# deeppowers/deeppowers

Hardware: AMD Instinct MI355X
Metric: ciphertext-mul/s (N=4096, 4 RNS limbs) (higher is better)
Workload: dtype u64

## Files before the change

### deeppowers_amd/csrc/ctx_tables.h

```cpp
#pragma once
#include <cstring>
#include <vector>

#include "devtables.h"
#include "ntt_core.h"
#include "ntt_quarters.h"
#include "tables.h"

namespace dpfhe {

static_assert(sizeof(TwShoup) == 16 && sizeof(TwFold) == 16 && sizeof(TwF64) == 16, "the twiddle slots of every class share one stride");
struct alignas(16) TwBytes { u64 lo, hi; };
constexpr size_t kTwSize = sizeof(TwBytes);

template <class Tw> inline TwBytes tw_bytes(const Tw& t) { static_assert(sizeof(Tw) == sizeof(TwBytes), "slot size"); TwBytes r; std::memcpy(&r, &t, sizeof r); return r; }
inline TwBytes class_tw(LimbClass k, u64 w, u64 q) {
    if (k == kClassFold) return tw_bytes(h_tw_fold(w, q));
    if (k == kClassFoldScaled) return tw_bytes(h_tw_fold_scaled(w, q, fold_scaled_shift(q)));
    if (k == kClassF64 || k == kClassF64Wide) return tw_bytes(h_make_tw<TwF64>(w, q));
    return tw_bytes(h_make_tw<TwShoup>(w, q));
}
inline InvLast<TwBytes> class_last(LimbClass k, u64 w_last, u64 w_ninv, u64 q) { return InvLast<TwBytes>{class_tw(k, w_last, q), class_tw(k, w_ninv, q)}; }
inline void pack_table(unsigned char* dst, const std::vector<u64>& words, LimbClass k, u64 q, int logn_tab, int loge) {
    std::vector<TwBytes> t(words.size());
// ... 34 lines not shown
        const u64 sinv = cls == kClassFoldScaled ? h_powmod((1ull << fold_scaled_shift(q)) % q, q - 2, q) : 1;
        reinterpret_cast<InvLast<TwBytes>*>(&blob[m.o_last2])[l] = class_last(cls, h_mulmod(t.w_last, sinv, q), h_mulmod(t.lc.ninv, sinv, q), q);
    }
    return blob;
}
template <class Arith>
inline DevTables<Arith> mixed_view(const unsigned char* b, const MixedLayout& m, size_t L) {
    typedef typename Arith::Tw Tw;
    DevTables<Arith> tb{};
    tb.lc = reinterpret_cast<const LimbConst*>(b + m.o_lc);
    tb.fwd = reinterpret_cast<const Tw*>(b + m.o_fwd); tb.inv = reinterpret_cast<const Tw*>(b + m.o_inv);
    tb.fwd4 = reinterpret_cast<const Tw*>(b + m.o_fwd4); tb.inv4 = reinterpret_cast<const Tw*>(b + m.o_inv4);
    tb.last = reinterpret_cast<const InvLast<Tw>*>(b + m.o_last);
    tb.last2 = reinterpret_cast<const InvLast<Tw>*>(b + m.o_last2);
    tb.n_sub = 1;
    tb.n_limbs = (int)L;
    return tb;
}
inline bool ctx_limb_classes(int log2n, const std::vector<HostLimbTables>& ht, bool fold, unsigned char limb_cls[16]) {
    if (fold || ht.size() > 16 || log2n < 8 || log2n > 14) return false;
    bool any_fast = false;
    for (size_t l = 0; l < ht.size(); ++l) { limb_cls[l] = (unsigned char)limb_class(ht[l].lc.q); any_fast = any_fast || limb_cls[l] != kClassShoup; }
    return any_fast;
}

struct CtxLayout {
    int log_n1, log_n2, loge_ntt;
    size_t n_sub, n2;
    bool split, two_geo, halves, quarters;
    size_t o_lc, o_fwd4, o_inv4, o_fwd, o_inv, o_last, o_top_fwd, o_top_inv, o_top_last, o_resc, o_hfwd, o_hinv, o_htop_fwd, o_htop_last,
           o_qfwd, o_qinv, o_qtop_fwd, o_qtop_inv, o_qtop_last, total;
};
inline CtxLayout ctx_layout(int log2n, size_t L, bool fold) {
    auto up = [](size_t x) { return (x + 255) & ~(size_t)255; };
    CtxLayout m;
    m.log_n1 = split_log_n1(log2n); m.log_n2 = log2n - m.log_n1;
    m.n_sub = (size_t)1 << m.log_n1; m.n2 = (size_t)1 << m.log_n2;
    m.loge_ntt = ntt_loge(m.log_n2);
    m.split = m.log_n1 > 0; m.two_geo = !m.split && m.loge_ntt != kFusedLoge;
    m.halves = log2n == 13 && fold;
    m.quarters = log2n == 14 && fold;
    const size_t n_sub = m.n_sub, tab = L * ((size_t)1 << log2n) * kTwSize;
    m.o_lc = 0; m.o_fwd4 = up(m.o_lc + L * sizeof(LimbConst)); m.o_inv4 = up(m.o_fwd4 + tab);
    m.o_fwd = m.two_geo ? up(m.o_inv4 + tab) : m.o_fwd4; m.o_inv = m.two_geo ? up(m.o_fwd + tab) : m.o_inv4;
    m.o_last = up(m.o_inv + tab); m.o_top_fwd = up(m.o_last + L * n_sub * 2 * kTwSize); m.o_top_inv = up(m.o_top_fwd + L * n_sub * kTwSize);
    m.o_top_last = up(m.o_top_inv + L * n_sub * kTwSize); m.o_resc = up(m.o_top_last + L * 2 * kTwSize);
// ... 86 lines not shown
```

### deeppowers_amd/csrc/devtables.h

```cpp
#pragma once
#include "modarith.h"

namespace dpfhe {

struct QuartersTop;

constexpr int ntt_loge(int ) { return 4; }
constexpr int kMaxLog2N = 16;
constexpr int kSplitLog2N2 = 12;
constexpr int split_log_n1(int log2n) { return log2n > 14 ? log2n - kSplitLog2N2 : 0; }
constexpr int kFusedLoge = 4;

template <class Tw>
struct InvLast {
    Tw w_last;
    Tw w_ninv;
};

template <class Arith>
struct DevTables {
    const typename Arith::Tw* fwd;
    const typename Arith::Tw* inv;
    const typename Arith::Tw* fwd4;
    const typename Arith::Tw* inv4;
    const typename Arith::Tw* top_fwd;
    const typename Arith::Tw* top_inv;
    const InvLast<typename Arith::Tw>* top_last;
    int n_sub;
    const typename Arith::Tw* hfwd;
    const typename Arith::Tw* hinv;
    const typename Arith::Tw* htop_fwd;
    const InvLast<typename Arith::Tw>* htop_last;
    const typename Arith::Tw* qfwd;
    const typename Arith::Tw* qinv;
    const struct QuartersTop* qtop_fwd;
    const typename Arith::Tw* qtop_inv;
    const InvLast<typename Arith::Tw>* qtop_last;
    const InvLast<typename Arith::Tw>* last;
    const InvLast<typename Arith::Tw>* last2;
    const LimbConst* lc;
    int n_limbs;
    int n_active;
    unsigned long long active_map;
};

template <class TB>
DPF_HD void block_item_limb(const TB& tb, size_t blk, size_t& item, int& limb) {
    if (tb.n_active) {
        item = blk / (unsigned)tb.n_active;
        limb = (int)((tb.active_map >> (4u * (unsigned)(blk % (unsigned)tb.n_active))) & 15u);
    } else {
        item = blk / (unsigned)tb.n_limbs;
        limb = (int)(blk % (unsigned)tb.n_limbs);
    }
}

struct MixedTables {
    const void* fwd;
    const void* inv;
    const void* last;
    const LimbConst* lc;
    int n_limbs;
// ... 12 lines not shown
```

### deeppowers_amd/csrc/dpfhe_cabi.hip

```cpp
#include <dlfcn.h>
#include <hip/hip_runtime.h>

#include <algorithm>
#include <atomic>
#include <cstdio>
#include <cstdlib>
#include <cstring>
#include <mutex>
#include <new>
#include <string>
#include <vector>

#include "../../include/dpfhe.h"
#include "base_ext.h"
#include "compact.h"
#include "ctx_tables.h"
#include "encode.h"
#include "expand.h"
#include "noise.h"
#include "plain_add.h"
#include "kernels_large.h"
#include "kernels_misc.h"
#include "launch.h"
#include "tables.h"
// ... 35 lines not shown
    return a0 < b0 + nb && b0 < a0 + na;
}
static inline bool overlaps(const uint64_t* a, size_t na, const uint64_t* b, size_t nb) { return overlaps_bytes(a, na * 8, b, nb * 8); }

static inline bool misaligned(const void* p) { return (reinterpret_cast<uintptr_t>(p) & 15) != 0; }
static const size_t kMaxGrid = 0x7fffffff;

struct dpfhe_ctx {
    uint32_t log2n = 0, n_limbs = 0;
    int device = 0;
    bool fold = false;
    int n_cu = 256;
    std::vector<uint64_t> moduli;
    uint64_t p_special = 0;
    void* d_blob = nullptr;
    const LimbConst* lc = nullptr;
    const RescaleConst* d_rescale = nullptr;
    DevTables<ShoupArith> shoup{};
    DevTables<FoldArith> foldt{};
    bool classes = false;
    int uniform_cls = kClassShoup;
    unsigned char limb_cls[16] = {};
    unsigned long long cls_map = 0;
    void* class_blob = nullptr;
    DevTables<FoldArith> cls_fold{};
    DevTables<F64Arith> cls_f64{};
    DevTables<FoldScaledArith> cls_fscaled{};
    DevTables<F64WideArith> cls_f64w{};
    DevTables<ShoupArith> cls_shoup{};
    MixedTables mixed{};
    struct ScratchArena { hipStream_t stream; u64* p; size_t words; uint64_t last_use; };
    std::vector<ScratchArena> scratch_arenas;
    uint64_t scratch_clock = 0;
    std::mutex scratch_mutex;
    std::atomic<int> ct_mul_variant{0};
    dpfhe_tune_info tune{};
    mutable std::mutex tune_mutex;
    std::atomic<size_t> scratch_limit_words{(size_t)1024 << 17};
};


static const char* const kCtMulVariantNames[kCtMulVariants] = {"quad", "dual"};
static const float kTuneMargin = 0.97f;

__global__ __launch_bounds__(256) void tune_fill_kernel(u64* __restrict__ p, size_t n) {
    for (size_t i = (size_t)blockIdx.x * 256 + threadIdx.x; i < n; i += (size_t)gridDim.x * 256)
// ... 161 lines not shown
    c->d_rescale = reinterpret_cast<const RescaleConst*>(d + lay.o_resc);
    if (fold) c->foldt = ctx_view<FoldArith>(d, lay, L);
    else c->shoup = ctx_view<ShoupArith>(d, lay, L);
    if (ctx_limb_classes((int)log2_n, ht, fold, c->limb_cls)) {
        const MixedLayout m = mixed_layout((int)log2_n, L);
        const std::vector<unsigned char> mb = build_class_blob((int)log2_n, ht, c->limb_cls);
        for (size_t l = 0; l < L; ++l) c->cls_map |= (unsigned long long)c->limb_cls[l] << (4 * l);
        if (int rc = upload(c->class_blob, mb, "dpfhe_ctx_create: class table upload")) return rc;
        const unsigned char* b = static_cast<const unsigned char*>(c->class_blob);
        c->cls_fold = mixed_view<FoldArith>(b, m, L);
        c->cls_f64 = mixed_view<F64Arith>(b, m, L);
        c->cls_fscaled = mixed_view<FoldScaledArith>(b, m, L);
        c->cls_f64w = mixed_view<F64WideArith>(b, m, L);
        c->cls_shoup = mixed_view<ShoupArith>(b, m, L);
        c->mixed.fwd = b + m.o_fwd; c->mixed.inv = b + m.o_inv; c->mixed.last = b + m.o_last;
        c->mixed.lc = reinterpret_cast<const LimbConst*>(b + m.o_lc);
        c->mixed.n_limbs = (int)L;
        c->mixed.cls_map = c->cls_map;
        c->classes = true;
        bool same = true;
        for (size_t l = 1; l < L; ++l) same = same && c->limb_cls[l] == c->limb_cls[0];
        if (same) c->uniform_cls = c->limb_cls[0];
    }
    tune_at_create(c);
    (void)hipSetDevice(prev);
    *out = c;
    return DPFHE_SUCCESS;
}

extern "C" int dpfhe_ctx_destroy(dpfhe_ctx* c) {
    if (!c) return DPFHE_SUCCESS;
    if (c->d_blob) (void)hipFree(c->d_blob);
    if (c->class_blob) (void)hipFree(c->class_blob);
    for (auto& a : c->scratch_arenas) if (a.p) (void)hipFree(a.p);
    delete c;
    return DPFHE_SUCCESS;
}
extern "C" int dpfhe_ctx_set_scratch_limit(dpfhe_ctx* c, size_t mib) {
    if (!c) return fail(DPFHE_INVALID_ARGUMENT, "dpfhe_ctx_set_scratch_limit", "null context");
    if (mib == 0 || mib > ((size_t)1 << 20)) return fail(DPFHE_INVALID_ARGUMENT, "dpfhe_ctx_set_scratch_limit", "limit must be in [1 MiB, 1 TiB]");
    c->scratch_limit_words.store(mib << 17, std::memory_order_relaxed);
    return DPFHE_SUCCESS;
}
extern "C" uint32_t dpfhe_ctx_log2n(const dpfhe_ctx* c) { return c ? c->log2n : 0; }
extern "C" uint32_t dpfhe_ctx_limbs(const dpfhe_ctx* c) { return c ? c->n_limbs : 0; }
extern "C" int dpfhe_ctx_uses_fold(const dpfhe_ctx* c) { return c && c->fold ? 1 : 0; }
extern "C" int dpfhe_ctx_limb_class(const dpfhe_ctx* c, uint32_t limb) {
    if (!c || limb >= c->n_limbs) return -1;
    if (c->classes) return (int)c->limb_cls[limb];
    return c->fold ? DPFHE_ARITH_FOLD : DPFHE_ARITH_SHOUP;
}
static_assert(DPFHE_ARITH_SHOUP == kClassShoup && DPFHE_ARITH_FOLD == kClassFold && DPFHE_ARITH_F64 == kClassF64 && DPFHE_ARITH_FOLD_SCALED == kClassFoldScaled &&
              DPFHE_ARITH_F64_WIDE == kClassF64Wide, "dpfhe.h <-> tables.h");

constexpr int kMatvecWpt2 = 2, kMatvecWpt4 = 1;
constexpr int kMatvecWd = 1;
// ... 1489 lines not shown
```

### deeppowers_amd/csrc/kernels.h

```cpp
#pragma once
#include <hip/hip_runtime.h>

#include "devtables.h"
#include "launch.h"
#include "ntt_core.h"
#include "ntt_top.h"

namespace dpfhe {

__device__ __forceinline__ void lds_barrier() { __syncthreads(); }
__device__ __forceinline__ void wave_sync() {
    __builtin_amdgcn_fence(__ATOMIC_ACQ_REL, "wavefront");
    __builtin_amdgcn_wave_barrier();
}
template <class G, int X, bool FWD>
__device__ __forceinline__ void exch_sync_before_write() {
    if constexpr (G::exch_wave_local(X)) {
        wave_sync();
    } else {
        constexpr bool first = FWD ? X == 0 : G::highest_cross_wave_exchange() == X;
        if constexpr (!first) lds_barrier();
    }
}
template <class G, int X>
// ... 509 lines not shown
        InvChain2<BI, B::NPH - 1, kInvIn>::run(tid, D0, D1, lds, lds + W, twi, last, lc);
        B::inv_canon(D0, lc);
        B::template store_top<true>(tid, D0, dst);
        B::inv_canon(D1, lc);
        B::template store_top<true>(tid, D1, dst + cstride);
        asm volatile("" : "+v"(tid));
        lds_barrier();
        InvChain<BI, B::NPH - 1, kInvIn>::run(tid, D2, lds, twi, last, lc);
        B::inv_canon(D2, lc);
        B::template store_top<true>(tid, D2, dst + 2 * cstride);
    }
}

constexpr int kTraceWords = 12;
template <bool TRACE>
__device__ __forceinline__ u64 trace_stamp(u64 dep) {
    u64 t = 0;
    if constexpr (TRACE) asm volatile("s_memrealtime %0\n\ts_waitcnt lgkmcnt(0)" : "=s"(t) : "v"(dep) : "memory");
    return t;
}
template <class Arith, int LOGN, int LOGE, bool TRACE = false, bool OUT_NTT = false>
__global__ __launch_bounds__(1 << (LOGN - LOGE), 2) void ct_mul_quad_kernel(u64* __restrict__ out3, const u64* __restrict__ a2,
                                                                         const u64* __restrict__ b2, DevTables<Arith> tb, u64* __restrict__ trace = nullptr) {
    typedef NttBody<Arith, LOGN, LOGE> B;
    static_assert(B::kLazyProducts && LOGE == kFusedLoge, "a policy with lazy products (ntt_core.h prod), fused twiddle layout");
    typedef NttBody<Arith, LOGN, LOGE, 0, kUnit, true> BI;
    constexpr bool kScaledProducts = Arith::kFoldCore && !Arith::kFold;
    constexpr int E = B::E, N = B::G::N, W = B::G::lds_words();
    __shared__ __attribute__((aligned(16))) u64 lds[2 * W];
    const int tid = threadIdx.x;
    const u64 ts0 = trace_stamp<TRACE>((u64)tid);
    const size_t L = (size_t)tb.n_limbs;
    size_t bi;
    int limb;
    block_item_limb(tb, blockIdx.x, bi, limb);
    const LimbConst lc = tb.lc[limb];
    const u64* src_a = a2 + ((bi * 2) * L + limb) * N;
    const u64* src_b = b2 + ((bi * 2) * L + limb) * N;
    u64* dst = out3 + ((bi * 3) * L + limb) * N;
    const size_t cstride = L * N;
    const InvLast<typename B::Tw> last = kScaledProducts ? tb.last2[limb] : tb.last[limb];
    constexpr int kInvIn = B::kProdInvIn;
    u64 x[E], y[E], z[E], w[E];
    const u64 ts_p = trace_stamp<TRACE>((u64)(uintptr_t)src_a ^ (u64)lc.q);
    B::template load_top<true>(tid, x, src_a);
    const u64 ts_x = trace_stamp<TRACE>((u64)tid);
    B::template load_top<true>(tid, y, src_b);
    B::template load_top<true>(tid, z, src_a + cstride);
    B::template load_top<true>(tid, w, src_b + cstride);
    const u64 ts_i = trace_stamp<TRACE>((u64)tid);
    const u64 ts1 = trace_stamp<TRACE>(x[0]);
    const u64 ts_xl = trace_stamp<TRACE>(x[E - 1]);
    FwdChain4<B, 0>::run(tid, x, y, z, w, lds, lds + W, tb.fwd4 + (size_t)limb * N, lc);
    B::prod_partner(y, lc);
    B::prod_partner(w, lc);
    const u64 ts2 = trace_stamp<TRACE>(w[E - 1]);
#pragma unroll
    for (int k = 0; k < E; ++k) {
        const u64 a0 = x[k], b0 = y[k], a1 = z[k], b1 = w[k];
        B::tensor(a0, a1, b0, b1, x[k], y[k], z[k], lc);
    }
    const u64 ts3 = trace_stamp<TRACE>(z[E - 1]);
    if constexpr (OUT_NTT) {
        static_assert(Arith::kFold && !TRACE, "the pinned primes (the products of a scaled-fold limb carry the scale twice)");
#pragma unroll
        for (int k = 0; k < E; ++k) { x[k] = FoldArith::canon_small(x[k], lc); y[k] = FoldArith::canon_small(y[k], lc); z[k] = FoldArith::canon_small(z[k], lc); }
        B::store_bot(tid, x, dst);
        B::store_bot(tid, y, dst + cstride);
        B::store_bot(tid, z, dst + 2 * cstride);
        return;
    }
    constexpr bool kNtStore = true;
    InvChain3<BI, B::NPH - 1, kInvIn>::run(tid, x, y, z, lds, lds + W, tb.inv4 + (size_t)limb * N, last, lc);
    const u64 ts4 = trace_stamp<TRACE>(z[E - 1]);
    B::inv_canon(x, lc);
    B::template store_top<kNtStore>(tid, x, dst);
    B::inv_canon(y, lc);
    B::template store_top<kNtStore>(tid, y, dst + cstride);
    B::inv_canon(z, lc);
    B::template store_top<kNtStore>(tid, z, dst + 2 * cstride);
    if constexpr (TRACE) {
        const u64 ts5 = trace_stamp<TRACE>((u64)tid);
        asm volatile("s_waitcnt vmcnt(0)" ::: "memory");
        const u64 ts6 = trace_stamp<TRACE>((u64)tid);
        if (tid == 0) {
            unsigned hw, xcc;
            asm volatile("s_getreg_b32 %0, hwreg(HW_REG_HW_ID)" : "=s"(hw));
            asm volatile("s_getreg_b32 %0, hwreg(HW_REG_XCC_ID)" : "=s"(xcc));
            u64* t = trace + (size_t)blockIdx.x * kTraceWords;
            t[0] = ts0; t[1] = ts1; t[2] = ts2; t[3] = ts3; t[4] = ts4; t[5] = ts5; t[6] = ts6;
            t[7] = (u64)hw | ((u64)xcc << 32);
            t[8] = ts_p; t[9] = ts_x; t[10] = ts_i; t[11] = ts_xl;
        }
    }
}

// ... 408 lines not shown
```

### deeppowers_amd/csrc/modarith.h

```cpp
#pragma once
#include <stdint.h>

#if defined(__HIPCC__)
#define DPF_HD __host__ __device__ __forceinline__
#else
#define DPF_HD inline __attribute__((always_inline))
#endif

namespace dpfhe {

typedef uint64_t u64;
typedef uint32_t u32;

#if defined(DPFHE_EMU_CHECK) && !defined(__HIPCC__)
extern long g_emu_overflows;
#define DPFHE_EMU_ASSERT(cond) do { if (!(cond)) ++g_emu_overflows; } while (0)
#else
#define DPFHE_EMU_ASSERT(cond) do { } while (0)
#endif

struct LimbConst {
    u64 q;
    u64 d;
    u64 ninv;
// ... 112 lines not shown
        DPFHE_EMU_ASSERT(((a | b | as | bs) >> 30) == 0);
        const u64 H = mad32(y1, bs, mad32(y0, b, 0));
        u32 two30 = 1u << 30;
#if defined(__HIP_DEVICE_COMPILE__)
        asm("s_mov_b32 %0, 0x40000000" : "=s"(two30));
#endif
        const u64 L = mad32(y1, as, mad32(y0, a, mad32((u32)H, two30, 0)));
        const u64 R = mad32((u32)(H >> 32), 4 * (u32)c.d, L);
        return reduce(R, c);
    }
    static DPF_HD u64 mul_tw_add(u64 y, const Tw& t, const LimbConst& c, u64 addend) {
        const u32 y0 = (u32)y, y1 = (u32)(y >> 32);
        const u32 a = (u32)t.w, b = (u32)(t.w >> 32), as = (u32)t.ws, bs = (u32)(t.ws >> 32);
        DPFHE_EMU_ASSERT(((a | b | as | bs) >> 30) == 0);
        DPFHE_EMU_ASSERT((unsigned __int128)addend + ((unsigned __int128)y0 << 30) + ((unsigned __int128)y1 << 30) + (1ull << 62) + (1ull << 54) < ((unsigned __int128)1 << 64));
        const u64 H = mad32(y1, bs, mad32(y0, b, 0));
        u32 two30 = 1u << 30;
#if defined(__HIP_DEVICE_COMPILE__)
        asm("s_mov_b32 %0, 0x40000000" : "=s"(two30));
#endif
        const u64 L = mad32(y1, as, mad32(y0, a, mad32((u32)H, two30, addend)));
        const u64 R = mad32((u32)(H >> 32), 4 * (u32)c.d, L);
        return reduce(R, c);
    }
    static DPF_HD Tw prod_tw(u64 b, const LimbConst& c) {
        DPFHE_EMU_ASSERT(b < (1ull << 60) + (1ull << 29));
        const u32 lo = (u32)b;
        u32 a = lo & 0x3fffffffu, bh = (u32)(b >> 30), t29 = (u32)(b >> 29), bl = lo & 0x1fffffffu;
#if defined(__HIP_DEVICE_COMPILE__)
        asm("" : "+v"(a), "+v"(bh), "+v"(t29), "+v"(bl));
#endif
        const u64 bs = add_hi32(mad32(t29, 2 * (u32)c.d, 0), bl);
        u32 as = (u32)bs & 0x3fffffffu, bsh = (u32)(bs >> 30);
#if defined(__HIP_DEVICE_COMPILE__)
        asm("" : "+v"(as), "+v"(bsh));
#endif
        Tw t;
        t.w = (u64)a | ((u64)bh << 32);
        t.ws = (u64)as | ((u64)bsh << 32);
        return t;
    }
    static DPF_HD bool ptw_fits(u32 y0, u32 y1, u32 a, u32 b, u32 as, u32 bs, u64 addend, u32 d) {
        typedef unsigned __int128 u128;
        const u128 H = (u128)y0 * b + (u128)y1 * bs;
        const u128 L = (u128)((u32)(u64)H) * (1u << 30) + (u128)y0 * a + (u128)y1 * as + addend;
        return (H >> 64) == 0 && ((L + (u128)(u32)((u64)H >> 32) * (4 * d)) >> 64) == 0;
// ... 153 lines not shown
```

### deeppowers_amd/csrc/ntt_core.h

```cpp
#pragma once
#include "modarith.h"

namespace dpfhe {

#if defined(DPFHE_EMU_CHECK) && !defined(__HIPCC__)
inline u64 chk_add(u64 a, u64 b) { if ((unsigned __int128)a + b >> 64) ++g_emu_overflows; return a + b; }
inline u64 chk_sub_add(u64 a, u64 b, u64 off) {
    __int128 v = (__int128)a - (__int128)b + (__int128)off;
    if (v < 0 || (v >> 64)) ++g_emu_overflows;
    return a - b + off;
}
inline u64 chk_shl1_add_sub(u64 a, u64 c, u64 s) {
    __int128 v = 2 * (__int128)a + (__int128)c - (__int128)s;
    if (v < 0 || (v >> 64) || ((unsigned __int128)2 * a + c) >> 64) ++g_emu_overflows;
    return shl1_add(a, c) - s;
}
#else
DPF_HD u64 chk_shl1_add_sub(u64 a, u64 c, u64 s) { return shl1_add(a, c) - s; }
DPF_HD u64 chk_add(u64 a, u64 b) { return a + b; }
DPF_HD u64 chk_sub_add(u64 a, u64 b, u64 off) { return a - b + off; }
#endif

struct Phase {
    int c;
    int b;
    int r;
};

constexpr int geo_nph(int logn, int loge) { return (logn + loge - 1) / loge; }
constexpr Phase geo_phase(int logn, int loge, int p) {
    int rem = logn, top = logn, r = 0;
    for (int i = 0; i <= p; ++i) {
        int left = geo_nph(logn, loge) - i;
        r = (rem + left - 1) / left;
        top = rem;
        rem -= r;
    }
    int b = top - r;
    int c = b < (logn - loge) ? b : (logn - loge);
    return Phase{c, b, r};
// ... 137 lines not shown
    int bnd[E] = {};
    for (int k = 0; k < E; ++k) bnd[k] = in_bound;
    for (int u = 0; u < r; ++u) {
        const int bit = 1 << (lb_top - u);
        for (int k = 0; k < E; ++k) {
            if (k & bit) continue;
            int A = bnd[k];
            const int Y = bnd[k | bit];
            if (A + Y / 4 + 1 > kFuseLimit || (u == r - 1 && A > kRedB && 2 * A + 2 * kUnit > out_cap)) { p.red_a[u][k] = true; A = kRedB; }
            bnd[k] = kRedB;
            bnd[k | bit] = 2 * A + 2 * kUnit;
        }
    }
    int mx = 0;
    for (int k = 0; k < E; ++k) {
        if (bnd[k] > out_cap) { p.red_end[k] = true; bnd[k] = kRedB; }
        p.out[k] = bnd[k];
        if (bnd[k] > mx) mx = bnd[k];
    }
    p.out_bound = mx;
    return p;
}

constexpr int kF64Red = kUnit / 2 + 1, kF64Tw = kUnit;
template <int LOGE>
struct F64CtPlan {
    bool red_y[LOGE][1 << LOGE];
    bool red_a[LOGE][1 << LOGE];
    bool red_end[1 << LOGE];
    int out_bound;
};
template <int LOGE>
constexpr F64CtPlan<LOGE> make_f64_ct_plan(int lb_top, int r, int in_bound, int out_cap, int cap) {
    F64CtPlan<LOGE> p{};
    constexpr int E = 1 << LOGE;
    int bnd[E] = {};
    for (int k = 0; k < E; ++k) bnd[k] = in_bound;
    for (int u = 0; u < r; ++u) {
        const int bit = 1 << (lb_top - u);
        for (int k = 0; k < E; ++k) {
            if (k & bit) continue;
            int A = bnd[k], Y = bnd[k | bit];
            if (Y > cap) { p.red_y[u][k] = true; Y = kF64Red; }
            if (A + kF64Tw > 4 * cap) { p.red_a[u][k] = true; A = kF64Red; }
            bnd[k] = bnd[k | bit] = A + kF64Tw;
        }
// ... 18 lines not shown
    int bnd[E] = {};
    for (int k = 0; k < E; ++k) bnd[k] = in_bound;
    for (int u = 0; u < r; ++u) {
        const int bit = 1 << (lb0 + u);
        for (int k = 0; k < E; ++k) {
            if (k & bit) continue;
            int bx = bnd[k], by = bnd[k | bit];
            if (bx + by > cap) {
                if (bx > kF64Red) { p.red[u][k] = true; bx = kF64Red; }
                if (by > kF64Red) { p.red[u][k | bit] = true; by = kF64Red; }
            }
            bnd[k] = (last_all_mul && u == r - 1) ? kF64Tw : bx + by;
            bnd[k | bit] = kF64Tw;
        }
    }
    for (int k = 0; k < E; ++k) {
        p.red_end[k] = bnd[k] > out_bound;
        if (p.red_end[k]) bnd[k] = kF64Red;
    }
    return p;
}

constexpr int kSubInvOut = 7 * kUnit;
template <class Arith, int LOGN, int LOGE, int SUB = 0, int FWD_IN = (SUB ? kCtfMid : kUnit), bool RAW_INV = false>
struct NttBody {
    typedef Geo<LOGN, LOGE> G;
    typedef typename Arith::Tw Tw;
    static constexpr int E = G::E, T = G::T, NPH = G::NPH;
    static_assert(FWD_IN >= kUnit && FWD_IN <= kCtfMid && (!SUB || FWD_IN == kCtfMid), "forward input bound: canonical ... the phase hand-over bound");

    static DPF_HD unsigned row_base(int k) {
        constexpr int kReach = 4096 / (T * 8) > 0 ? 4096 / (T * 8) : 1;
        unsigned b = (unsigned)(k / kReach * kReach) * T;
#if defined(__HIP_DEVICE_COMPILE__)
        asm("" : "+s"(b));
#endif
        return b;
    }
    template <bool NT, class V>
    static DPF_HD V ld_stream(const V* p) {
#if defined(__HIP_DEVICE_COMPILE__)
        if (NT) return __builtin_nontemporal_load(p);
#endif
        return *p;
    }
    template <bool NT, class V>
    static DPF_HD void st_stream(V* p, V v) {
#if defined(__HIP_DEVICE_COMPILE__)
        if (NT) { __builtin_nontemporal_store(v, p); return; }
#endif
        *p = v;
    }
// ... 230 lines not shown
        int in = kUnit;
        for (int i = 0; i < P; ++i) {
            const Phase pi = G::phase(i);
            in = make_f64_ct_plan<LOGE>(pi.b - pi.c + pi.r - 1, pi.r, in, 2 * kF64Cap, kF64Cap).out_bound;
        }
        return make_f64_ct_plan<LOGE>(ph.b - ph.c + ph.r - 1, ph.r, in, (P == NPH - 1) ? kF64Cap : 2 * kF64Cap, kF64Cap);
    }
    template <int P, int IN>
    static constexpr F64GsPlan<LOGE> f64_gs_plan() {
        constexpr Phase ph = G::phase(P);
        constexpr int mid = kF64Cap / 2 > 2 * kUnit ? 2 * kUnit : kF64Cap / 2;
        return make_f64_gs_plan<LOGE>(ph.b - ph.c, ph.r, (P == NPH - 1) ? IN : mid, (P == 0) ? kF64Cap : mid, P == 0, kF64Cap);
    }
    template <int P>
    static constexpr CtfPlan<LOGE> ctf_plan() {
        constexpr Phase ph = G::phase(P);
        int in = FWD_IN;
        for (int i = 0; i < P; ++i) {
            const Phase pi = G::phase(i);
            in = make_ctf_plan<LOGE>(pi.b - pi.c + pi.r - 1, pi.r, in, kCtfMid).out_bound;
        }
        return make_ctf_plan<LOGE>(ph.b - ph.c + ph.r - 1, ph.r, in, (P == NPH - 1) ? kWord : kCtfMid);
    }
    static constexpr int kFwdOutBound = Arith::kFoldCore ? ctf_plan<NPH - 1>().out_bound : Arith::kF64 ? f64_ct_plan<NPH - 1>().out_bound : 4 * kUnit;
    static_assert(!Arith::kFoldCore || kFwdOutBound <= kLimitPartner, "lazy forward outputs must satisfy mul60's bound");

    static constexpr bool kConverts = Arith::kF64 || (Arith::kFoldCore && !Arith::kFold);
    static_assert(!kConverts || !SUB, "the halves form is FoldArith's");

    static DPF_HD void enter(u64 (&x)[E], const LimbConst& lc) {
        if constexpr (kConverts) {
#pragma clang loop unroll(full)
            for (int k = 0; k < E; ++k) x[k] = Arith::enter(x[k], lc);
        }
    }
    template <int P>
    static DPF_HD void fwd_phase_r(u64 (&x)[E], const TwRegs& twr, const LimbConst& lc_in) {
        constexpr Phase ph = G::phase(P);
        const auto& lc = Arith::ntt_lc(lc_in);
        if constexpr (P == 0) enter(x, lc_in);
        const u64 two_q = 2 * lc.q;
        if constexpr (Arith::kF64) {
            constexpr F64CtPlan<LOGE> plan = f64_ct_plan<P>();
            const double q = Arith::qd(lc), qi = Arith::qinv(lc);
#pragma clang loop unroll(full)
            for (int u = 0; u < ph.r; ++u) {
                const int lb = ph.b + ph.r - 1 - u - ph.c;
#pragma clang loop unroll(full)
                for (int k = 0; k < E; ++k) {
                    if (k & (1 << lb)) continue;
                    const int kk = k | (1 << lb);
                    const Tw& w = twr[u][k >> (lb + 1)];
                    double a = Arith::f(x[k]), y = Arith::f(x[kk]);
                    if (plan.red_a[u][k]) a = Arith::reduce(a, q, qi);
                    if (plan.red_y[u][k]) y = Arith::reduce(y, q, qi);
                    const double t = Arith::mulmod(y, w.w, w.wq, q);
                    x[k] = Arith::b(a + t);
                    x[kk] = Arith::b(a - t);
                }
            }
#pragma clang loop unroll(full)
            for (int k = 0; k < E; ++k)
                if (plan.red_end[k]) x[k] = Arith::b(Arith::reduce(Arith::f(x[k]), q, qi));
        } else if constexpr (Arith::kFoldCore) {
            constexpr CtfPlan<LOGE> plan = ctf_plan<P>();
#pragma clang loop unroll(full)
            for (int u = 0; u < ph.r; ++u) {
                const int lb = ph.b + ph.r - 1 - u - ph.c;
#pragma clang loop unroll(full)
                for (int k = 0; k < E; ++k) {
                    if (k & (1 << lb)) continue;
                    const int kk = k | (1 << lb);
                    u64 a = x[k];
                    if (plan.red_a[u][k]) a = FoldArith::reduce(a, lc);
                    const u64 s = FoldArith::mul_tw_add(x[kk], twr[u][k >> (lb + 1)], lc, a);
                    x[k] = s;
                    x[kk] = chk_shl1_add_sub(a, two_q, s);
                }
            }
#pragma clang loop unroll(full)
            for (int k = 0; k < E; ++k)
                if (plan.red_end[k]) x[k] = FoldArith::reduce(x[k], lc);
        } else {
#pragma clang loop unroll(full)
            for (int u = 0; u < ph.r; ++u) {
                const int lb = ph.b + ph.r - 1 - u - ph.c;
#pragma clang loop unroll(full)
                for (int k = 0; k < E; ++k) {
                    if (k & (1 << lb)) continue;
                    const u64 a = csub(x[k], two_q);
                    const u64 t = Arith::mul_tw(x[k | (1 << lb)], twr[u][k >> (lb + 1)], lc);
                    x[k] = a + t;
                    x[k | (1 << lb)] = a - t + two_q;
                }
            }
        }
    }
    template <int P>
    static DPF_HD void fwd_phase(int tid, u64 (&x)[E], const Tw* tw, const LimbConst& lc) {
        TwRegs twr;
        load_tw<P, true>(tid, tw, twr);
        fwd_phase_r<P>(x, twr, lc);
    }
    static DPF_HD void fwd_canon(u64 (&x)[E], const LimbConst& lc_in) {
        const auto& lc = Arith::ntt_lc(lc_in);
        if constexpr (Arith::kF64) {
#pragma clang loop unroll(full)
            for (int k = 0; k < E; ++k) x[k] = Arith::leave(x[k], lc);
        } else if constexpr (Arith::kFoldCore) {
            constexpr CtfPlan<LOGE> plan = ctf_plan<NPH - 1>();
#pragma clang loop unroll(full)
            for (int k = 0; k < E; ++k) {
                x[k] = plan.out[k] <= kRedB ? FoldArith::canon_small(x[k], lc) : FoldArith::canon(x[k], lc);
                if constexpr (kConverts) x[k] = Arith::leave(x[k], lc_in);
            }
        } else {
#pragma clang loop unroll(full)
            for (int k = 0; k < E; ++k) x[k] = csub(csub(x[k], 2 * lc.q), lc.q);
        }
    }

    static DPF_HD void fwd_reduce_partner(u64 (&x)[E], const LimbConst& lc_in) {
        static_assert(Arith::kFoldCore, "fold policies only");
        const auto& lc = Arith::ntt_lc(lc_in);
        constexpr CtfPlan<LOGE> plan = ctf_plan<NPH - 1>();
#pragma clang loop unroll(full)
        for (int k = 0; k < E; ++k)
            if (plan.out[k] > kRedB) x[k] = FoldArith::reduce(x[k], lc);
    }

    static constexpr bool kLazyProducts = Arith::kFoldCore || Arith::kF64;
    static constexpr int kProdInvIn = Arith::kF64 ? 2 * kUnit : kRedB;
    static_assert(!Arith::kF64 || kFwdOutBound <= kF64Cap, "F64ArithT: |a b / q| <= |a| / 2 must stay below 2^50 for the quotient estimate of a lazy product");
    static DPF_HD void prod_partner(u64 (&y)[E], const LimbConst& lc) {
        if constexpr (Arith::kF64) {
            const double q = Arith::qd(lc), qi = Arith::qinv(lc);
#pragma clang loop unroll(full)
            for (int k = 0; k < E; ++k) y[k] = Arith::b(Arith::reduce(Arith::f(y[k]), q, qi));
        } else fwd_reduce_partner(y, lc);
    }
    static DPF_HD u64 prod(u64 a, u64 b, const LimbConst& lc) {
        if constexpr (Arith::kF64) {
            const double x = Arith::f(a), y = Arith::f(b), q = Arith::qd(lc);
            const double p = x * y;
            const double e = __builtin_fma(x, y, -p);
            const double h = Arith::rint_mul(p, Arith::qinv(lc));
            return Arith::b(__builtin_fma(-h, q, p) + e);
        } else return FoldArith::mul60(a, b, (u32)lc.d);
    }
    static DPF_HD u64 prod_add(u64 p, u64 r) {
        if constexpr (Arith::kF64) return Arith::b(Arith::f(p) + Arith::f(r));
// ... 35 lines not shown
                const int lb = pos - ph.c;
                const bool last = (pos == LOGN - 1);
#pragma clang loop unroll(full)
                for (int k = 0; k < E; ++k) {
                    if (k & (1 << lb)) continue;
                    const int kk = k | (1 << lb);
                    double a = Arith::f(x[k]), b = Arith::f(x[kk]);
                    if (plan.red[u][k]) a = Arith::reduce(a, q, qi);
                    if (plan.red[u][kk]) b = Arith::reduce(b, q, qi);
                    const double s = a + b, dlt = a - b;
                    if (last) {
                        x[k] = Arith::b(Arith::mulmod(s, w_ninv.w, w_ninv.wq, q));
                        x[kk] = Arith::b(Arith::mulmod(dlt, w_last.w, w_last.wq, q));
                    } else {
                        const Tw& w = twr[u][k >> (lb + 1)];
                        x[k] = Arith::b(s);
                        x[kk] = Arith::b(Arith::mulmod(dlt, w.w, w.wq, q));
                    }
                }
            }
#pragma clang loop unroll(full)
            for (int k = 0; k < E; ++k)
                if (plan.red_end[k]) x[k] = Arith::b(Arith::reduce(Arith::f(x[k]), q, qi));
        } else {
            constexpr GsPlan<LOGE> plan = gs_plan<P, IN>();
            const u64 q = lc.q, two_q = 2 * lc.q;
#pragma clang loop unroll(full)
            for (int u = 0; u < ph.r; ++u) {
                const int pos = ph.b + u;
                const int lb = pos - ph.c;
                const bool last = (pos == LOGN - 1) && !SUB;
#pragma clang loop unroll(full)
                for (int k = 0; k < E; ++k) {
                    if (k & (1 << lb)) continue;
                    const int kk = k | (1 << lb);
                    u64 a = x[k], b = x[kk];
                    u64 s, dlt;
                    if constexpr (Arith::kFoldCore) {
                        if (plan.red[u][k]) a = FoldArith::reduce(a, lc);
                        if (plan.red[u][kk]) b = FoldArith::reduce(b, lc);
                        s = chk_add(a, b);
                        dlt = chk_sub_add(a, b, (u64)plan.off[u][k] * q);
                    } else {
                        s = csub(a + b, two_q);
                        dlt = a - b + two_q;
                    }
// ... 43 lines not shown
```

### deeppowers_amd/csrc/tables.h

```cpp
#pragma once
#include <vector>

#include "modarith.h"

namespace dpfhe {

typedef unsigned __int128 u128;

inline u64 h_mulmod(u64 a, u64 b, u64 q) { return (u64)((u128)a * b % q); }
inline u64 h_powmod(u64 b, u64 e, u64 q) {
    u64 r = 1;
    b %= q;
    for (; e; e >>= 1) {
        if (e & 1) r = h_mulmod(r, b, q);
        b = h_mulmod(b, b, q);
    }
    return r;
}
inline bool h_is_prime(u64 n) {
    if (n < 2) return false;
    const u64 bases[12] = {2, 3, 5, 7, 11, 13, 17, 19, 23, 29, 31, 37};
    for (u64 p : bases) {
        if (n == p) return true;
        if (n % p == 0) return false;
// ... 3 lines not shown
    while (!(d & 1)) { d >>= 1; ++r; }
    for (u64 a : bases) {
        u64 x = h_powmod(a, d, n);
        if (x == 1 || x == n - 1) continue;
        bool witness = true;
        for (int i = 1; i < r && witness; ++i) {
            x = h_mulmod(x, x, n);
            if (x == n - 1) witness = false;
        }
        if (witness) return false;
    }
    return true;
}
inline u64 h_shoup(u64 w, u64 q) { return (u64)(((u128)w << 64) / q); }
inline u32 h_brv(u32 x, int bits) {
    u32 r = 0;
    for (int i = 0; i < bits; ++i) { r = (r << 1) | (x & 1); x >>= 1; }
    return r;
}

inline TwFold h_tw_fold(u64 w, u64 q) {
    const u64 ws = (u64)(((u128)w << 32) % q), m30 = (1ull << 30) - 1;
    return TwFold{(w & m30) | ((w >> 30) << 32), (ws & m30) | ((ws >> 30) << 32)};
}

template <class Tw> inline Tw h_make_tw(u64 w, u64 q);
template <> inline TwFold h_make_tw<TwFold>(u64 w, u64 q) { return h_tw_fold(w, q); }
template <> inline TwShoup h_make_tw<TwShoup>(u64 w, u64 q) { return TwShoup{w, (u64)(((u128)w << 64) / q)}; }
template <> inline TwF64 h_make_tw<TwF64>(u64 w, u64 q) { return TwF64{(double)w, (double)w / (double)q}; }

enum LimbClass { kClassShoup = 0, kClassFold = 1, kClassF64 = 2, kClassFoldScaled = 3, kClassF64Wide = 4, kLimbClasses = 5 };
inline int h_bit_length(u64 v) { int b = 0; while (v) { ++b; v >>= 1; } return b; }
inline int fold_scaled_shift(u64 q) {
    const int k = h_bit_length(q);
    if (k < 48 || k > 59) return 0;
    const u64 d0 = (1ull << k) - q;
    return (d0 << (60 - k)) < (1ull << 24) ? 60 - k : 0;
}
inline bool f64_eligible(u64 q) { return q < (1ull << F64Arith::kMaxBits); }
inline LimbClass limb_class(u64 q) {
    if (q < (1ull << 60) && ((1ull << 60) - q) < (1ull << 24)) return kClassFold;
    if (f64_eligible(q)) return kClassF64;
    if (fold_scaled_shift(q)) return kClassFoldScaled;
    if (q < (1ull << F64WideArith::kMaxBits)) return kClassF64Wide;
    return kClassShoup;
}
// ... 76 lines not shown
```

Measured before the change: 2.435 million.

## Add lazy 29-bit split twiddle path for fold-prime N=4096 ct-mul NTTs

Adds a second twiddle encoding that splits each twiddle at bit 29 instead of 30, with a multiply-accumulate (mul_tw29_add) that folds the butterfly addend into the twiddle product and skips the final reduce. Compile-time lazy reduction plans for the forward (CT) and inverse (GS) stages decide where reductions are needed, aiming to remove most per-butterfly modular reductions in the fused ct_mul kernel at N=4096. New tables are built and uploaded at context creation for fold-class limbs. The cost is extra device memory, more complex bound reasoning, and possible register pressure.

```diff
diff --git a/deeppowers_amd/csrc/ctx_tables.h b/deeppowers_amd/csrc/ctx_tables.h
--- a/deeppowers_amd/csrc/ctx_tables.h
+++ b/deeppowers_amd/csrc/ctx_tables.h
@@ -80,6 +80,43 @@
     bool any_fast = false;
     for (size_t l = 0; l < ht.size(); ++l) { limb_cls[l] = (unsigned char)limb_class(ht[l].lc.q); any_fast = any_fast || limb_cls[l] != kClassShoup; }
     return any_fast;
+}
+
+constexpr int kLazy29Log2N = 12;
+struct Lazy29Layout { size_t o_fwd, o_inv, o_last, total; };
+inline Lazy29Layout lazy29_layout(size_t L) {
+    auto up = [](size_t x) { return (x + 255) & ~(size_t)255; };
+    const size_t tab = L * ((size_t)1 << kLazy29Log2N) * kTwSize;
+    Lazy29Layout m;
+    m.o_fwd = 0; m.o_inv = up(tab); m.o_last = up(m.o_inv + tab); m.total = up(m.o_last + L * 2 * kTwSize);
+    return m;
+}
+inline std::vector<unsigned char> build_lazy29_blob(int log2n, const std::vector<HostLimbTables>& ht, const std::vector<bool>& fold_limb) {
+    bool any = false;
+    for (size_t l = 0; l < ht.size(); ++l) any = any || fold_limb[l];
+    if (log2n != kLazy29Log2N || !any) return {};
+    const size_t L = ht.size(), n = (size_t)1 << log2n;
+    const Lazy29Layout m = lazy29_layout(L);
+    std::vector<unsigned char> blob(m.total, 0);
+    auto pack29 = [&](size_t off, const std::vector<u64>& words, u64 q) {
+        std::vector<TwBytes> t(words.size());
+        for (size_t i = 0; i < words.size(); ++i) t[i] = tw_bytes(h_tw_fold29(words[i], q));
+        permute_window0(t, log2n, kFusedLoge, geo_perm_stages(log2n, kFusedLoge));
+        std::memcpy(&blob[off], t.data(), t.size() * kTwSize);
+    };
+    for (size_t l = 0; l < L; ++l) {
+        if (!fold_limb[l]) continue;
+        const HostLimbTables& t = ht[l];
+        const u64 q = t.lc.q;
+        pack29(m.o_fwd + l * n * kTwSize, t.rp, q);
+        pack29(m.o_inv + l * n * kTwSize, t.irp, q);
+        reinterpret_cast<InvLast<TwBytes>*>(&blob[m.o_last])[l] = InvLast<TwBytes>{tw_bytes(h_tw_fold29(t.w_last, q)), tw_bytes(h_tw_fold29(t.lc.ninv, q))};
+    }
+    return blob;
+}
+inline void lazy29_view(DevTables<FoldArith>& tb, const unsigned char* d, const Lazy29Layout& m) {
+    tb.fwd29 = reinterpret_cast<const TwFold*>(d + m.o_fwd); tb.inv29 = reinterpret_cast<const TwFold*>(d + m.o_inv);
+    tb.last29 = reinterpret_cast<const InvLast<TwFold>*>(d + m.o_last);
 }
 
 struct CtxLayout {
diff --git a/deeppowers_amd/csrc/devtables.h b/deeppowers_amd/csrc/devtables.h
--- a/deeppowers_amd/csrc/devtables.h
+++ b/deeppowers_amd/csrc/devtables.h
@@ -38,6 +38,9 @@
     const InvLast<typename Arith::Tw>* qtop_last;
     const InvLast<typename Arith::Tw>* last;
     const InvLast<typename Arith::Tw>* last2;
+    const typename Arith::Tw* fwd29;
+    const typename Arith::Tw* inv29;
+    const InvLast<typename Arith::Tw>* last29;
     const LimbConst* lc;
     int n_limbs;
     int n_active;
diff --git a/deeppowers_amd/csrc/dpfhe_cabi.hip b/deeppowers_amd/csrc/dpfhe_cabi.hip
--- a/deeppowers_amd/csrc/dpfhe_cabi.hip
+++ b/deeppowers_amd/csrc/dpfhe_cabi.hip
@@ -81,6 +81,7 @@
     int uniform_cls = kClassShoup;
     unsigned char limb_cls[16] = {};
     unsigned long long cls_map = 0;
+    void* lazy29_blob = nullptr;
     void* class_blob = nullptr;
     DevTables<FoldArith> cls_fold{};
     DevTables<F64Arith> cls_f64{};
@@ -288,6 +289,15 @@
         for (size_t l = 1; l < L; ++l) same = same && c->limb_cls[l] == c->limb_cls[0];
         if (same) c->uniform_cls = c->limb_cls[0];
     }
+    {
+        std::vector<bool> fold_limb(L);
+        for (size_t l = 0; l < L; ++l) fold_limb[l] = fold || (c->classes && c->limb_cls[l] == kClassFold);
+        const std::vector<unsigned char> lb = build_lazy29_blob((int)log2_n, ht, fold_limb);
+        if (!lb.empty()) {
+            if (int rc = upload(c->lazy29_blob, lb, "dpfhe_ctx_create: lazy table upload")) return rc;
+            lazy29_view(fold ? c->foldt : c->cls_fold, static_cast<const unsigned char*>(c->lazy29_blob), lazy29_layout(L));
+        }
+    }
     tune_at_create(c);
     (void)hipSetDevice(prev);
     *out = c;
@@ -298,6 +308,7 @@
     if (!c) return DPFHE_SUCCESS;
     if (c->d_blob) (void)hipFree(c->d_blob);
     if (c->class_blob) (void)hipFree(c->class_blob);
+    if (c->lazy29_blob) (void)hipFree(c->lazy29_blob);
     for (auto& a : c->scratch_arenas) if (a.p) (void)hipFree(a.p);
     delete c;
     return DPFHE_SUCCESS;
diff --git a/deeppowers_amd/csrc/kernels.h b/deeppowers_amd/csrc/kernels.h
--- a/deeppowers_amd/csrc/kernels.h
+++ b/deeppowers_amd/csrc/kernels.h
@@ -555,13 +555,14 @@
 template <class Arith, int LOGN, int LOGE, bool TRACE = false, bool OUT_NTT = false>
 __global__ __launch_bounds__(1 << (LOGN - LOGE), 2) void ct_mul_quad_kernel(u64* __restrict__ out3, const u64* __restrict__ a2,
                                                                          const u64* __restrict__ b2, DevTables<Arith> tb, u64* __restrict__ trace = nullptr) {
-    typedef NttBody<Arith, LOGN, LOGE> B;
+    constexpr bool kLazy29 = Arith::kFold && LOGN == 12;
+    typedef NttBody<Arith, LOGN, LOGE, 0, kUnit, false, kLazy29> B;
     static_assert(B::kLazyProducts && LOGE == kFusedLoge, "a policy with lazy products (ntt_core.h prod), fused twiddle layout");
-    typedef NttBody<Arith, LOGN, LOGE, 0, kUnit, true> BI;
+    typedef NttBody<Arith, LOGN, LOGE, 0, kUnit, true, kLazy29> BI;
     constexpr bool kScaledProducts = Arith::kFoldCore && !Arith::kFold;
     constexpr int E = B::E, N = B::G::N, W = B::G::lds_words();
     __shared__ __attribute__((aligned(16))) u64 lds[2 * W];
-    const int tid = threadIdx.x;
+    int tid = threadIdx.x;
     const u64 ts0 = trace_stamp<TRACE>((u64)tid);
     const size_t L = (size_t)tb.n_limbs;
     size_t bi;
@@ -572,8 +573,11 @@
     const u64* src_b = b2 + ((bi * 2) * L + limb) * N;
     u64* dst = out3 + ((bi * 3) * L + limb) * N;
     const size_t cstride = L * N;
-    const InvLast<typename B::Tw> last = kScaledProducts ? tb.last2[limb] : tb.last[limb];
+    const InvLast<typename B::Tw> last = kLazy29 ? tb.last29[limb] : kScaledProducts ? tb.last2[limb] : tb.last[limb];
+    const typename B::Tw* const tw_fwd = (kLazy29 ? tb.fwd29 : tb.fwd4) + (size_t)limb * N;
+    const typename B::Tw* const tw_inv = (kLazy29 ? tb.inv29 : tb.inv4) + (size_t)limb * N;
     constexpr int kInvIn = B::kProdInvIn;
+    static_assert(!kLazy29 || (B::template lazy_fwd_reductions<>() == 40 && BI::template lazy_inv_reductions<kInvIn>() == 55), "lazy plans of the N = 4096 geometry");
     u64 x[E], y[E], z[E], w[E];
     const u64 ts_p = trace_stamp<TRACE>((u64)(uintptr_t)src_a ^ (u64)lc.q);
     B::template load_top<true>(tid, x, src_a);
@@ -584,7 +588,8 @@
     const u64 ts_i = trace_stamp<TRACE>((u64)tid);
     const u64 ts1 = trace_stamp<TRACE>(x[0]);
     const u64 ts_xl = trace_stamp<TRACE>(x[E - 1]);
-    FwdChain4<B, 0>::run(tid, x, y, z, w, lds, lds + W, tb.fwd4 + (size_t)limb * N, lc);
+    if constexpr (kLazy29) { asm volatile("" : "+v"(tid)); __builtin_assume(tid >= 0 && tid < B::T); }
+    FwdChain4<B, 0>::run(tid, x, y, z, w, lds, lds + W, tw_fwd, lc);
     B::prod_partner(y, lc);
     B::prod_partner(w, lc);
     const u64 ts2 = trace_stamp<TRACE>(w[E - 1]);
@@ -604,7 +609,7 @@
         return;
     }
     constexpr bool kNtStore = true;
-    InvChain3<BI, B::NPH - 1, kInvIn>::run(tid, x, y, z, lds, lds + W, tb.inv4 + (size_t)limb * N, last, lc);
+    InvChain3<BI, B::NPH - 1, kInvIn>::run(tid, x, y, z, lds, lds + W, tw_inv, last, lc);
     const u64 ts4 = trace_stamp<TRACE>(z[E - 1]);
     B::inv_canon(x, lc);
     B::template store_top<kNtStore>(tid, x, dst);
diff --git a/deeppowers_amd/csrc/modarith.h b/deeppowers_amd/csrc/modarith.h
--- a/deeppowers_amd/csrc/modarith.h
+++ b/deeppowers_amd/csrc/modarith.h
@@ -158,6 +158,26 @@
         const u64 L = mad32(y1, as, mad32(y0, a, mad32((u32)H, two30, addend)));
         const u64 R = mad32((u32)(H >> 32), 4 * (u32)c.d, L);
         return reduce(R, c);
+    }
+    static DPF_HD u64 mul_tw29_add(u64 y, const Tw& t, const LimbConst& c, u64 addend) {
+        const u32 y0 = (u32)y, y1 = (u32)(y >> 32);
+        const u32 a = (u32)t.w, b = (u32)(t.w >> 32), as = (u32)t.ws, bs = (u32)(t.ws >> 32);
+        DPFHE_EMU_ASSERT(((a | as) >> 29) == 0 && ((b | bs) >> 31) == 0);
+        DPFHE_EMU_ASSERT(tw29_fits(y0, y1, a, b, as, bs, addend, (u32)c.d));
+        const u64 H = mad32(y1, bs, mad32(y0, b, 0));
+        u32 two29 = 1u << 29;
+#if defined(__HIP_DEVICE_COMPILE__)
+        asm("s_mov_b32 %0, 0x20000000" : "=s"(two29));
+#endif
+        const u64 L = mad32(y1, as, mad32(y0, a, mad32((u32)H, two29, addend)));
+        return mad32((u32)(H >> 32), 2 * (u32)c.d, L);
+    }
+    static DPF_HD u64 mul_tw29(u64 y, const Tw& t, const LimbConst& c) { return mul_tw29_add(y, t, c, 0); }
+    static DPF_HD bool tw29_fits(u32 y0, u32 y1, u32 a, u32 b, u32 as, u32 bs, u64 addend, u32 d) {
+        typedef unsigned __int128 u128;
+        const u128 H = (u128)y0 * b + (u128)y1 * bs;
+        const u128 L = (u128)((u32)(u64)H) * (1u << 29) + (u128)y0 * a + (u128)y1 * as + addend;
+        return (H >> 64) == 0 && (L >> 64) == 0 && ((L + (u128)(u32)((u64)H >> 32) * (2 * d)) >> 64) == 0;
     }
     static DPF_HD Tw prod_tw(u64 b, const LimbConst& c) {
         DPFHE_EMU_ASSERT(b < (1ull << 60) + (1ull << 29));
diff --git a/deeppowers_amd/csrc/ntt_core.h b/deeppowers_amd/csrc/ntt_core.h
--- a/deeppowers_amd/csrc/ntt_core.h
+++ b/deeppowers_amd/csrc/ntt_core.h
@@ -15,7 +15,13 @@
     if (v < 0 || (v >> 64) || ((unsigned __int128)2 * a + c) >> 64) ++g_emu_overflows;
     return shl1_add(a, c) - s;
 }
+inline u64 chk_lazy_diff(u64 a, u64 c, u64 s) {
+    __int128 v = 2 * (__int128)a + (__int128)c - (__int128)s;
+    if (v < 0 || (v >> 64)) ++g_emu_overflows;
+    return shl1_add(a, c) - s;
+}
 #else
+DPF_HD u64 chk_lazy_diff(u64 a, u64 c, u64 s) { return shl1_add(a, c) - s; }
 DPF_HD u64 chk_shl1_add_sub(u64 a, u64 c, u64 s) { return shl1_add(a, c) - s; }
 DPF_HD u64 chk_add(u64 a, u64 b) { return a + b; }
 DPF_HD u64 chk_sub_add(u64 a, u64 b, u64 off) { return a - b + off; }
@@ -199,6 +205,88 @@
     return p;
 }
 
+constexpr int kLazy29B = 4 * kUnit + kUnit / 8 + 1;
+constexpr int kCtf29Mid = 14 * kUnit;
+constexpr int kGs29Mid = 6 * kUnit + kUnit / 4;
+
+template <int LOGE>
+struct Ctf29Plan {
+    bool red_a[LOGE][1 << LOGE];
+    int K[LOGE][1 << LOGE];
+    bool red_end[1 << LOGE];
+    int out[1 << LOGE];
+    int out_bound;
+    int n_red;
+};
+template <int LOGE>
+constexpr Ctf29Plan<LOGE> make_ctf29_plan(int lb_top, int r, int in_bound, int out_cap) {
+    Ctf29Plan<LOGE> p{};
+    constexpr int E = 1 << LOGE;
+    int bnd[E] = {};
+    for (int k = 0; k < E; ++k) bnd[k] = in_bound;
+    for (int u = 0; u < r; ++u) {
+        const int bit = 1 << (lb_top - u);
+        for (int k = 0; k < E; ++k) {
+            if (k & bit) continue;
+            int A = bnd[k];
+            const int P = kLazy29B + (bnd[k | bit] + 7) / 8;
+            const int K = (P + kUnit - 1) / kUnit;
+            bool red = P + A > kWord || A + K * kUnit > kWord;
+            if (!red && u == r - 1 && A > kRedB && (P + A > out_cap || A + K * kUnit > out_cap) && P + kRedB <= out_cap && kRedB + K * kUnit <= out_cap) red = true;
+            if (red) { p.red_a[u][k] = true; A = kRedB; ++p.n_red; }
+            p.K[u][k] = K;
+            bnd[k] = P + A;
+            bnd[k | bit] = A + K * kUnit;
+        }
+    }
+    for (int k = 0; k < E; ++k) {
+        if (bnd[k] > out_cap) { p.red_end[k] = true; bnd[k] = kRedB; ++p.n_red; }
+        p.out[k] = bnd[k];
+        if (bnd[k] > p.out_bound) p.out_bound = bnd[k];
+    }
+    return p;
+}
+
+template <int LOGE>
+struct Gs29Plan {
+    bool red[LOGE][1 << LOGE];
+    int off[LOGE][1 << LOGE];
+    bool red_end[1 << LOGE];
+    int out_bound;
+    int n_red;
+};
+template <int LOGE>
+constexpr Gs29Plan<LOGE> make_gs29_plan(int lb0, int r, int in_bound, int out_cap, bool last, int ninv_shift) {
+    Gs29Plan<LOGE> p{};
+    constexpr int E = 1 << LOGE;
+    int bnd[E] = {};
+    for (int k = 0; k < E; ++k) bnd[k] = in_bound;
+    for (int u = 0; u < r; ++u) {
+        const int bit = 1 << (lb0 + u);
+        const bool fin = last && u == r - 1;
+        const int sum_cap = fin ? kWord - kUnit / 8 : kWord;
+        for (int k = 0; k < E; ++k) {
+            if (k & bit) continue;
+            int bx = bnd[k], by = bnd[k | bit];
+            for (int pass = 0; pass < 2; ++pass) {
+                if (bx + by <= sum_cap && bx + (by + kUnit - 1) / kUnit * kUnit <= kWord) break;
+                if (bx >= by && bx > kRedB) { p.red[u][k] = true; bx = kRedB; ++p.n_red; }
+                else { p.red[u][k | bit] = true; by = kRedB; ++p.n_red; }
+            }
+            const int offq = (by + kUnit - 1) / kUnit;
+            p.off[u][k] = offq;
+            bnd[k] = fin ? kUnit + ((bx + by) >> ninv_shift) + 2 : bx + by;
+            bnd[k | bit] = fin ? kRedB : kLazy29B + (bx + offq * kUnit + 7) / 8;
+            if (fin) ++p.n_red;
+        }
+    }
+    for (int k = 0; k < E; ++k) {
+        if (bnd[k] > out_cap) { p.red_end[k] = true; bnd[k] = kRedB; ++p.n_red; }
+        if (bnd[k] > p.out_bound) p.out_bound = bnd[k];
+    }
+    return p;
+}
+
 constexpr int kF64Red = kUnit / 2 + 1, kF64Tw = kUnit;
 template <int LOGE>
 struct F64CtPlan {
@@ -263,12 +351,13 @@
 }
 
 constexpr int kSubInvOut = 7 * kUnit;
-template <class Arith, int LOGN, int LOGE, int SUB = 0, int FWD_IN = (SUB ? kCtfMid : kUnit), bool RAW_INV = false>
+template <class Arith, int LOGN, int LOGE, int SUB = 0, int FWD_IN = (SUB ? kCtfMid : kUnit), bool RAW_INV = false, bool LAZY29 = false>
 struct NttBody {
     typedef Geo<LOGN, LOGE> G;
     typedef typename Arith::Tw Tw;
     static constexpr int E = G::E, T = G::T, NPH = G::NPH;
     static_assert(FWD_IN >= kUnit && FWD_IN <= kCtfMid && (!SUB || FWD_IN == kCtfMid), "forward input bound: canonical ... the phase hand-over bound");
+    static_assert(!LAZY29 || (Arith::kFold && !SUB), "the lazy plans are the pinned primes', one-piece transforms only");
 
     static DPF_HD unsigned row_base(int k) {
         constexpr int kReach = 4096 / (T * 8) > 0 ? 4096 / (T * 8) : 1;
@@ -545,8 +634,26 @@
         }
         return make_ctf_plan<LOGE>(ph.b - ph.c + ph.r - 1, ph.r, in, (P == NPH - 1) ? kWord : kCtfMid);
     }
-    static constexpr int kFwdOutBound = Arith::kFoldCore ? ctf_plan<NPH - 1>().out_bound : Arith::kF64 ? f64_ct_plan<NPH - 1>().out_bound : 4 * kUnit;
-    static_assert(!Arith::kFoldCore || kFwdOutBound <= kLimitPartner, "lazy forward outputs must satisfy mul60's bound");
+    template <int P>
+    static constexpr Ctf29Plan<LOGE> ctf29_plan() {
+        constexpr Phase ph = G::phase(P);
+        int in = FWD_IN;
+        for (int i = 0; i < P; ++i) {
+            const Phase pi = G::phase(i);
+            in = make_ctf29_plan<LOGE>(pi.b - pi.c + pi.r - 1, pi.r, in, kCtf29Mid).out_bound;
+        }
+        return make_ctf29_plan<LOGE>(ph.b - ph.c + ph.r - 1, ph.r, in, (P == NPH - 1) ? kWord : kCtf29Mid);
+    }
+    template <int P, int IN>
+    static constexpr Gs29Plan<LOGE> gs29_plan() {
+        constexpr Phase ph = G::phase(P);
+        return make_gs29_plan<LOGE>(ph.b - ph.c, ph.r, (P == NPH - 1) ? IN : kGs29Mid, (P == 0) ? 3 * kUnit / 2 : kGs29Mid, P == 0, LOGN);
+    }
+    template <int P = 0> static constexpr int lazy_fwd_reductions() { if constexpr (P < NPH) return ctf29_plan<P>().n_red + lazy_fwd_reductions<P + 1>(); else return 0; }
+    template <int IN, int P = 0> static constexpr int lazy_inv_reductions() { if constexpr (P < NPH) return gs29_plan<P, IN>().n_red + lazy_inv_reductions<IN, P + 1>(); else return 0; }
+    template <bool L = LAZY29> static constexpr int fwd_out_bound_fold() { if constexpr (L) return ctf29_plan<NPH - 1>().out_bound; else return ctf_plan<NPH - 1>().out_bound; }
+    static constexpr int kFwdOutBound = Arith::kFoldCore ? fwd_out_bound_fold<>() : Arith::kF64 ? f64_ct_plan<NPH - 1>().out_bound : 4 * kUnit;
+    static_assert(!Arith::kFoldCore || kFwdOutBound <= (LAZY29 ? kWord : kLimitPartner), "lazy forward outputs must satisfy mul60's bound (LAZY29: fit a word)");
 
     static constexpr bool kConverts = Arith::kF64 || (Arith::kFoldCore && !Arith::kFold);
     static_assert(!kConverts || !SUB, "the halves form is FoldArith's");
@@ -585,6 +692,25 @@
 #pragma clang loop unroll(full)
             for (int k = 0; k < E; ++k)
                 if (plan.red_end[k]) x[k] = Arith::b(Arith::reduce(Arith::f(x[k]), q, qi));
+        } else if constexpr (LAZY29) {
+            constexpr Ctf29Plan<LOGE> plan = ctf29_plan<P>();
+#pragma clang loop unroll(full)
+            for (int u = 0; u < ph.r; ++u) {
+                const int lb = ph.b + ph.r - 1 - u - ph.c;
+#pragma clang loop unroll(full)
+                for (int k = 0; k < E; ++k) {
+                    if (k & (1 << lb)) continue;
+                    const int kk = k | (1 << lb);
+                    u64 a = x[k];
+                    if (plan.red_a[u][k]) a = FoldArith::reduce(a, lc);
+                    const u64 s = FoldArith::mul_tw29_add(x[kk], twr[u][k >> (lb + 1)], lc, a);
+                    x[k] = s;
+                    x[kk] = chk_lazy_diff(a, (u64)plan.K[u][k] * lc.q, s);
+                }
+            }
+#pragma clang loop unroll(full)
+            for (int k = 0; k < E; ++k)
+                if (plan.red_end[k]) x[k] = FoldArith::reduce(x[k], lc);
         } else if constexpr (Arith::kFoldCore) {
             constexpr CtfPlan<LOGE> plan = ctf_plan<P>();
 #pragma clang loop unroll(full)
@@ -630,6 +756,9 @@
         if constexpr (Arith::kF64) {
 #pragma clang loop unroll(full)
             for (int k = 0; k < E; ++k) x[k] = Arith::leave(x[k], lc);
+        } else if constexpr (LAZY29) {
+#pragma clang loop unroll(full)
+            for (int k = 0; k < E; ++k) x[k] = FoldArith::canon(x[k], lc);
         } else if constexpr (Arith::kFoldCore) {
             constexpr CtfPlan<LOGE> plan = ctf_plan<NPH - 1>();
 #pragma clang loop unroll(full)
@@ -646,10 +775,17 @@
     static DPF_HD void fwd_reduce_partner(u64 (&x)[E], const LimbConst& lc_in) {
         static_assert(Arith::kFoldCore, "fold policies only");
         const auto& lc = Arith::ntt_lc(lc_in);
-        constexpr CtfPlan<LOGE> plan = ctf_plan<NPH - 1>();
-#pragma clang loop unroll(full)
-        for (int k = 0; k < E; ++k)
-            if (plan.out[k] > kRedB) x[k] = FoldArith::reduce(x[k], lc);
+        if constexpr (LAZY29) {
+            constexpr Ctf29Plan<LOGE> plan = ctf29_plan<NPH - 1>();
+#pragma clang loop unroll(full)
+            for (int k = 0; k < E; ++k)
+                if (plan.out[k] > kRedB) x[k] = FoldArith::reduce(x[k], lc);
+        } else {
+            constexpr CtfPlan<LOGE> plan = ctf_plan<NPH - 1>();
+#pragma clang loop unroll(full)
+            for (int k = 0; k < E; ++k)
+                if (plan.out[k] > kRedB) x[k] = FoldArith::reduce(x[k], lc);
+        }
     }
 
     static constexpr bool kLazyProducts = Arith::kFoldCore || Arith::kF64;
@@ -731,6 +867,35 @@
 #pragma clang loop unroll(full)
             for (int k = 0; k < E; ++k)
                 if (plan.red_end[k]) x[k] = Arith::b(Arith::reduce(Arith::f(x[k]), q, qi));
+        } else if constexpr (LAZY29) {
+            constexpr Gs29Plan<LOGE> plan = gs29_plan<P, IN>();
+            const u64 q = lc.q;
+#pragma clang loop unroll(full)
+            for (int u = 0; u < ph.r; ++u) {
+                const int pos = ph.b + u;
+                const int lb = pos - ph.c;
+                const bool last = (pos == LOGN - 1);
+#pragma clang loop unroll(full)
+                for (int k = 0; k < E; ++k) {
+                    if (k & (1 << lb)) continue;
+                    const int kk = k | (1 << lb);
+                    u64 a = x[k], b = x[kk];
+                    if (plan.red[u][k]) a = FoldArith::reduce(a, lc);
+                    if (plan.red[u][kk]) b = FoldArith::reduce(b, lc);
+                    const u64 s = chk_add(a, b);
+                    const u64 dlt = chk_sub_add(a, b, (u64)plan.off[u][k] * q);
+                    if (last) {
+                        x[k] = FoldArith::mul_ninv(s, lc, LOGN);
+                        x[kk] = FoldArith::reduce(FoldArith::mul_tw29(dlt, w_last, lc), lc);
+                    } else {
+                        x[k] = s;
+                        x[kk] = FoldArith::mul_tw29(dlt, twr[u][k >> (lb + 1)], lc);
+                    }
+                }
+            }
+#pragma clang loop unroll(full)
+            for (int k = 0; k < E; ++k)
+                if (plan.red_end[k]) x[k] = FoldArith::reduce(x[k], lc);
         } else {
             constexpr GsPlan<LOGE> plan = gs_plan<P, IN>();
             const u64 q = lc.q, two_q = 2 * lc.q;
diff --git a/deeppowers_amd/csrc/tables.h b/deeppowers_amd/csrc/tables.h
--- a/deeppowers_amd/csrc/tables.h
+++ b/deeppowers_amd/csrc/tables.h
@@ -49,6 +49,11 @@
 inline TwFold h_tw_fold(u64 w, u64 q) {
     const u64 ws = (u64)(((u128)w << 32) % q), m30 = (1ull << 30) - 1;
     return TwFold{(w & m30) | ((w >> 30) << 32), (ws & m30) | ((ws >> 30) << 32)};
+}
+
+inline TwFold h_tw_fold29(u64 w, u64 q) {
+    const u64 ws = (u64)(((u128)w << 32) % q), m29 = (1ull << 29) - 1;
+    return TwFold{(w & m29) | ((w >> 29) << 32), (ws & m29) | ((ws >> 29) << 32)};
 }
 
 template <class Tw> inline Tw h_make_tw(u64 w, u64 q);
```

Measured after the change: 2.603 million, median of 6. 1.07x the previous value.
